# SinclaM/ray-tracer-challenge

Measured on AMD Instinct MI355X. Metric: Mrays/sec (primary+secondary), scenes/cover.json 1920x1080 depth 5, higher is better.
Workload: dtype f64

## Files before the change

### ray-tracer-challenge_amd/csrc/rtc_kernels.hip

```cpp
#include "rtc_device.h"

#include <type_traits>

#if defined(RTC_PROFILE) && defined(RTC_PROFILE_LITE)
#define RTC_STAMP(sec)                                                     \
  do {                                                                     \
    if ((sec) == 7) prof_t = __builtin_amdgcn_s_memtime();                 \
    (void)prof_sec;                                                        \
  } while (0)
#define RTC_COUNT(slot) do { } while (0)
#define RTC_HIST_BEGIN() do { } while (0)
#define RTC_HIST_END(kind) do { } while (0)
#elif defined(RTC_PROFILE)
#define RTC_STAMP(sec)                                                     \
  do {                                                                     \
    const unsigned long long now_ = __builtin_amdgcn_s_memtime();          \
    prof_acc[prof_sec] += now_ - prof_t;                                   \
    prof_t = now_;                                                         \
    prof_sec = (sec);                                                      \
  } while (0)
#define RTC_COUNT(slot)                                                                 \
  do {                                                                                  \
    prof2[slot] += 1ull;                                                                \
    prof2[(slot) + 1] += static_cast<unsigned long long>(__builtin_popcountll(__ballot(true))); \
// ... 26 lines not shown
    if (__builtin_amdgcn_mbcnt_hi(static_cast<uint32_t>(__ballot(true) >> 32), __builtin_amdgcn_mbcnt_lo(static_cast<uint32_t>(__ballot(true)), 0u)) == 0u) \
      rtc_prof_counts[threadIdx.x >> 6][slot] += n_;                                                                   \
  } while (0)
#define RTC_WALK_ADD(slot, n) RTC_PROF_ADD_(slot, n)
#define RTC_AUX_ADD(slot, n) RTC_PROF_ADD_(8 + (slot), n)
#define RTC_KIND_ADD(slot, n) RTC_PROF_ADD_(16 + (slot), n)
#define RTC_CUBE_ADD(slot, n) RTC_PROF_ADD_(40 + (slot), n)
#else
#define RTC_WALK_ADD(slot, n) do { } while (0)
#define RTC_AUX_ADD(slot, n) do { } while (0)
#define RTC_KIND_ADD(slot, n) do { } while (0)
#define RTC_CUBE_ADD(slot, n) do { } while (0)
#endif

#ifdef RTC_PROFILE
__shared__ uint32_t rtc_oob_avail[6];
__device__ __forceinline__ bool rtc_in_bounds(uint32_t kind, bool ok) {
  if (!ok) atomicAdd(&rtc_prof_stats->oob[kind], 1ull);
  return ok;
}
#define RTC_IN_BOUNDS(kind, ok) rtc_in_bounds(kind, ok)
#define RTC_CHECK_INDEX(kind, i, n) (rtc_in_bounds(kind, (i) < (n)) ? (i) : 0u)
#define RTC_AVAIL(k) rtc_oob_avail[k]
#else
#define RTC_IN_BOUNDS(kind, ok) true
#define RTC_CHECK_INDEX(kind, i, n) (i)
#endif

#ifndef RTC_EXPERIMENT
#define RTC_EXPERIMENT 0
#endif

#ifndef RTC_ROOT_NODE_IN_REC
#define RTC_ROOT_NODE_IN_REC 1
#endif
#ifndef RTC_ALL_SOLID_FORM
#define RTC_ALL_SOLID_FORM 1
#endif
#ifndef RTC_CULL_HALF_STEP
#define RTC_CULL_HALF_STEP 1
#endif
#ifndef RTC_PLANE_EARLY_OUT
#define RTC_PLANE_EARLY_OUT 1
#endif
#ifndef RTC_ROOM_EARLY_OUT
#define RTC_ROOM_EARLY_OUT 1
#endif
#ifndef RTC_CUBE_BEHIND_EARLY_OUT
#define RTC_CUBE_BEHIND_EARLY_OUT 1
#endif
#ifndef RTC_SPECULAR_SKIP
#define RTC_SPECULAR_SKIP 1
#endif
#ifndef RTC_CONTAINERS_SOLIDS
#define RTC_CONTAINERS_SOLIDS 1
#endif
#ifndef RTC_SETPRIO
#define RTC_SETPRIO 1
#endif
#ifndef RTC_PRIO_DEAL
#define RTC_PRIO_DEAL 3
#endif
#ifndef RTC_PRIO_WORK
#define RTC_PRIO_WORK 1
#endif
#ifndef RTC_PRIO_CULL
#define RTC_PRIO_CULL 0
#endif
#ifndef RTC_PRIO_NODE
#define RTC_PRIO_NODE 0
#endif
#ifndef RTC_PRIO_CULL_SPHERES
#define RTC_PRIO_CULL_SPHERES 3
#endif
#if RTC_SETPRIO
#define RTC_PRIO_PHASE(x) __builtin_amdgcn_s_setprio(x)
#else
#define RTC_PRIO_PHASE(x) ((void)0)
#endif
#ifndef RTC_LB2
#define RTC_LB2 2
#endif

namespace {

constexpr double kInf = __builtin_huge_val();

struct Ray {
  double ox, oy, oz, dx, dy, dz;
};

__device__ __forceinline__ double zmax(double a, double b) { return __builtin_fmax(a, b); }
__device__ __forceinline__ double zmin(double a, double b) { return __builtin_fmin(a, b); }

__device__ __forceinline__ double row_pt(const double* __restrict__ m, double x, double y, double z) {
  return ((m[0] * x + m[1] * y) + m[2] * z) + m[3];
}
__device__ __forceinline__ double row_vec(const double* __restrict__ m, double x, double y, double z) {
  return (m[0] * x + m[1] * y) + m[2] * z;
}

__device__ __forceinline__ Ray xform_ray(const double* __restrict__ m, const Ray& r) {
  Ray o;
  o.ox = row_pt(m + 0, r.ox, r.oy, r.oz);
  o.oy = row_pt(m + 4, r.ox, r.oy, r.oz);
  o.oz = row_pt(m + 8, r.ox, r.oy, r.oz);
// ... 1012 lines not shown
                                                   const char* __restrict__ az, const RayB& rb) {
  const Float2 nx = *reinterpret_cast<const Float2*>(ax), fx = *reinterpret_cast<const Float2*>(ax + 8);
  const Float2 ny = *reinterpret_cast<const Float2*>(ay), fy = *reinterpret_cast<const Float2*>(ay + 8);
  const Float2 nz = *reinterpret_cast<const Float2*>(az), fz = *reinterpret_cast<const Float2*>(az + 8);
  const Float2 tnx = __builtin_elementwise_fma(nx, Float2(rb.ix), Float2(rb.cnx)), tny = __builtin_elementwise_fma(ny, Float2(rb.iy), Float2(rb.cny)),
               tnz = __builtin_elementwise_fma(nz, Float2(rb.iz), Float2(rb.cnz));
  const Float2 tfx = __builtin_elementwise_fma(fx, Float2(rb.ix), Float2(rb.cfx)), tfy = __builtin_elementwise_fma(fy, Float2(rb.iy), Float2(rb.cfy)),
               tfz = __builtin_elementwise_fma(fz, Float2(rb.iz), Float2(rb.cfz));
  uint32_t kept = 0u;
#pragma unroll
  for (int e = 0; e < 2; ++e) {
    const float tn = fmaxf(fmaxf(tnx[e], tny[e]), tnz[e]), tf = fminf(fminf(tfx[e], tfy[e]), tfz[e]);
    bool culled = fmaxf(tn, rb.t_lo) > fminf(tf, rb.t_hi);
    if constexpr (GROUPS) {
      const float line_only = (*reinterpret_cast<const Float2*>(pair + 72))[e];
      culled = line_only != 0.0f ? tn > tf : culled;
    }
    kept |= culled ? 0u : (1u << e);
  }
  return kept;
}

template <class V, bool GROUPS>
__device__ __forceinline__ uint32_t roots_kept_box4(const char* __restrict__ pair, const char* __restrict__ ax, const char* __restrict__ ay,
                                                    const char* __restrict__ az, const RayB& rb) {
  constexpr uint32_t NEXT = sizeof(RootBoxPair);
  const Float2 nx[2] = {*reinterpret_cast<const Float2*>(ax), *reinterpret_cast<const Float2*>(ax + NEXT)};
  const Float2 fx[2] = {*reinterpret_cast<const Float2*>(ax + 8), *reinterpret_cast<const Float2*>(ax + NEXT + 8)};
  const Float2 ny[2] = {*reinterpret_cast<const Float2*>(ay), *reinterpret_cast<const Float2*>(ay + NEXT)};
  const Float2 fy[2] = {*reinterpret_cast<const Float2*>(ay + 8), *reinterpret_cast<const Float2*>(ay + NEXT + 8)};
  const Float2 nz[2] = {*reinterpret_cast<const Float2*>(az), *reinterpret_cast<const Float2*>(az + NEXT)};
  const Float2 fz[2] = {*reinterpret_cast<const Float2*>(az + 8), *reinterpret_cast<const Float2*>(az + NEXT + 8)};
  uint32_t kept = 0u;
#pragma unroll
  for (int r = 0; r < 2; ++r) {
    const Float2 tnx = __builtin_elementwise_fma(nx[r], Float2(rb.ix), Float2(rb.cnx)), tny = __builtin_elementwise_fma(ny[r], Float2(rb.iy), Float2(rb.cny)),
                 tnz = __builtin_elementwise_fma(nz[r], Float2(rb.iz), Float2(rb.cnz));
    const Float2 tfx = __builtin_elementwise_fma(fx[r], Float2(rb.ix), Float2(rb.cfx)), tfy = __builtin_elementwise_fma(fy[r], Float2(rb.iy), Float2(rb.cfy)),
                 tfz = __builtin_elementwise_fma(fz[r], Float2(rb.iz), Float2(rb.cfz));
#pragma unroll
    for (int e = 0; e < 2; ++e) {
      const float tn = fmaxf(fmaxf(tnx[e], tny[e]), tnz[e]), tf = fminf(fminf(tfx[e], tfy[e]), tfz[e]);
      bool culled = fmaxf(tn, rb.t_lo) > fminf(tf, rb.t_hi);
      if constexpr (GROUPS) {
        const float line_only = (*reinterpret_cast<const Float2*>(pair + r * NEXT + 72))[e];
        culled = line_only != 0.0f ? tn > tf : culled;
      }
      kept |= culled ? 0u : (1u << (2 * r + e));
    }
  }
  return kept;
}

template <class V>
__device__ __forceinline__ void motion_root(V&, uint32_t) {}

template <bool CSG, int WORLD, class V, int TRAV = RTC_LDS_TRAV, bool BOX = true, bool MOTION = false>
__device__ __forceinline__ void trace(const DevScene& S, const RootRec* __restrict__ recs,
                                      const CullTables& cull, const Ray& ray, V& vis, unsigned& overflow,
                                      uint32_t* lds_stack, const uint32_t member = 0u, const uint32_t stride = 1u,
                                      const double* __restrict__ disp = nullptr, const double tm = 0.0) {
  constexpr bool SIMPLE = WORLD == 2, FLAT = WORLD >= 1;
  static_assert(!MOTION || WORLD == 0, "the motion kernels walk the general world");
  constexpr bool kSolids = SIMPLE && RTC_CONTAINERS_SOLIDS && V::kBehindOnly;
  const auto rf = [&]() {
    if constexpr (BOX) {
      RayB b = ray_box(ray, S, vis);
      if constexpr (kSolids) b.t_lo = -1.0002e-4f;
      return b;
    } else {
      return ray_f32(ray, S.cull_cmax);
    }
  }();
  const uint32_t n_bounded = S.n_roots - S.n_root_planes;
  for (uint32_t base = 0; base < S.n_roots; base += 64u) {
    const uint32_t n = min(64u, S.n_roots - base);
    const uint32_t nc = n_bounded > base ? min(n, n_bounded - base) : 0u;
    unsigned long long mine = 0ull;
    RTC_PRIO_PHASE(BOX ? RTC_PRIO_CULL : RTC_PRIO_CULL_SPHERES);
    if (BOX && FLAT && stride == 1u) {
      if constexpr (BOX) {
        const char* block = reinterpret_cast<const char*>(cull.box + (base >> 1));
        const char* ax = block + rf.onx;
        const char* ay = block + rf.ony;
        const char* az = block + rf.onz;
#if RTC_CULL_HALF_STEP
        const uint32_t whole = (nc & 3u) > 2u ? nc : (nc & ~3u);
#else
        const uint32_t whole = nc;
#endif
#ifdef RTC_PROFILE
        const bool reads_ok = RTC_IN_BOUNDS(RTC_OOB_ROOTS, (base >> 1) + 2u * ((whole + 3u) >> 2) + (whole < nc ? 1u : 0u) <= RTC_AVAIL(2));
#else
        constexpr bool reads_ok = true;
#endif
#pragma unroll 1
        for (uint32_t first = 0; reads_ok && first < whole; first += 4u) {
          const uint32_t k = roots_kept_box4<V, !FLAT>(block, ax, ay, az, rf);
          mine |= static_cast<unsigned long long>(k) << first;
          block += 2u * sizeof(RootBoxPair);
          ax += 2u * sizeof(RootBoxPair);
          ay += 2u * sizeof(RootBoxPair);
          az += 2u * sizeof(RootBoxPair);
        }
#if RTC_CULL_HALF_STEP
        if (reads_ok && whole < nc) mine |= static_cast<unsigned long long>(roots_kept_box<V, !FLAT>(block, ax, ay, az, rf)) << whole;
#endif
      }
    } else {
      for (uint32_t i = 4u * member; i < nc; i += 4u * stride) {
#ifdef RTC_PROFILE
        if (!RTC_IN_BOUNDS(RTC_OOB_ROOTS, ((base + i) >> 1) + ((BOX && !(i + 2u < nc)) ? 1u : 2u) <= RTC_AVAIL(BOX ? 2 : 1))) continue;
#endif
        unsigned long long k;
        if constexpr (BOX) {
          const char* const p0 = reinterpret_cast<const char*>(cull.box + ((base + i) >> 1));
          const char* const p1 = p0 + sizeof(RootBoxPair);
          k = roots_kept_box<V, !FLAT>(p0, p0 + rf.onx, p0 + rf.ony, p0 + rf.onz, rf);
          if (i + 2u < nc) k |= roots_kept_box<V, !FLAT>(p1, p1 + rf.onx, p1 + rf.ony, p1 + rf.onz, rf) << 2;
        } else {
          const RootCullPair p0 = cull.sphere[(base + i) >> 1], p1 = cull.sphere[((base + i) >> 1) + 1u];
          k = roots_kept<V, !FLAT, kSolids>(p0, rf) | (roots_kept<V, !FLAT, kSolids>(p1, rf) << 2);
        }
        mine |= k << i;
      }
    }
    if (nc < 64u) mine &= (1ull << nc) - 1ull;
    if (nc < n) {
      unsigned long long planes = (n < 64u ? (1ull << n) - 1ull : ~0ull) & ~((1ull << nc) - 1ull);
      if (stride != 1u) {
        unsigned long long own = 0xFull << (4u * member);
        if (stride == 4u) own |= own << 16;
        own |= own << 32;
        planes &= own;
      }
      mine |= planes;
    }
    RTC_PRIO_PHASE(RTC_PRIO_WORK);
    auto range = [&](uint32_t lo, uint32_t hi) -> unsigned long long {
      const uint32_t a = max(lo, base) - base, b = min(max(hi, base), base + 64u) - base;
      const unsigned long long below_b = b >= 64u ? ~0ull : (1ull << b) - 1ull;
      const unsigned long long below_a = a >= 64u ? ~0ull : (1ull << a) - 1ull;
      return below_b & ~below_a;
    };
#if defined(RTC_PROFILE) && !defined(RTC_PROFILE_LITE)
    uint32_t cube_tests = 0u, cube_neg = 0u, cube_pred = 0u;
#endif
    constexpr bool kCubeBehind = SIMPLE && BOX && V::kAnyHit && V::kFrontOnly && RTC_CUBE_BEHIND_EARLY_OUT;
    auto leaf_of_kind = [&](auto kind_tag, const uint32_t root) {
      constexpr uint32_t KIND = decltype(kind_tag)::value;
      const RootRec& R = recs[RTC_CHECK_INDEX(RTC_OOB_ROOTS, root, RTC_AVAIL(0))];
      const uint32_t kf = R.kind_flags;
      const Ray lr = xform_ray(R.inv, ray);
      const CylParams cy{0.0, 0.0, false};
      const uint32_t leaf = R.index, shadow = (kf >> 8) & 1u, material = R.material;
      vis.set_root(root);
      if constexpr (KIND == 2u && V::kAnyHit && RTC_ROOM_EARLY_OUT) {
        if ((kf & RTC_ROOT_ROOM) && segment_stays_inside_cube(lr, vis.t_limit())) return;
      }
#if defined(RTC_PROFILE) && !defined(RTC_PROFILE_LITE)
      if constexpr (KIND == 2u) {
        double c_tmin, c_tmax;
        cube_slab(lr, c_tmin, c_tmax);
        const bool neg = c_tmax < 0.0, pred = cube_entirely_behind(lr);
        constexpr uint32_t K = V::kAnyHit ? 6u : (V::kBehindOnly ? 12u : 0u);
        RTC_CUBE_ADD(K + 0u, __builtin_popcountll(__ballot(true)));
        RTC_CUBE_ADD(K + 1u, __builtin_popcountll(__ballot(neg)));
        RTC_CUBE_ADD(K + 2u, __builtin_popcountll(__ballot(pred)));
        RTC_CUBE_ADD(K + 3u, 1);
        cube_neg += neg ? 1u : 0u;
        cube_pred += pred ? 1u : 0u;
        cube_tests += 1u;
      }
#endif
      if constexpr (KIND == 2u && kCubeBehind) {
        if (cube_entirely_behind(lr)) return;
      }
      if constexpr (KIND == 1u && V::kFrontOnly && RTC_PLANE_EARLY_OUT) {
        if (__builtin_fabs(lr.dy) > 1e-5) {
          const double ao = __builtin_fabs(lr.oy), ad = __builtin_fabs(lr.dy);
          const bool negative = ((lr.oy > 0.0) == (lr.dy > 0.0)) & (ao >= 1e-290) & (ad <= 1e10);
          const bool beyond = ao > (vis.t_limit() * ad) * (1.0 + 1e-12);
          if (!(negative | beyond)) vis.entry(leaf, shadow, material, -lr.oy / lr.dy, 0.0, 0.0);
        }
      } else if constexpr (KIND == 1u && kSolids) {
        if (__builtin_fabs(lr.dy) > 1e-5 && (lr.oy > 0.0) == (lr.dy > 0.0)) vis.entry(leaf, shadow, material, -lr.oy / lr.dy, 0.0, 0.0);
      } else {
        leaf_entries<SIMPLE>(KIND, cy, nullptr, lr, [&](double t, double u, double v) { vis.entry(leaf, shadow, material, t, u, v); });
      }
    };
    auto leaves_of_kind = [&](auto kind_tag, unsigned long long m) {
      while (m != 0ull && !vis.done()) {
        const uint32_t bit = static_cast<uint32_t>(__builtin_ctzll(m));
        m &= m - 1ull;
        if constexpr (V::kBehindOnly) RTC_AUX_ADD(4, 1);
        leaf_of_kind(kind_tag, base + bit);
      }
    };
    if constexpr (FLAT) {
      const uint32_t k1 = S.n_root_spheres, k2 = k1 + S.n_root_cubes;
      if (stride == 1u) {
        const uint32_t p1 = base + n;
        for (uint32_t root = base + nc; root < p1; ++root) {
          if (__all(vis.done())) break;
          if constexpr (V::kBehindOnly) RTC_AUX_ADD(4, 1);
          if (!vis.done()) leaf_of_kind(std::integral_constant<uint32_t, 1u>{}, root);
        }

      } else {
        leaves_of_kind(std::integral_constant<uint32_t, 1u>{}, mine & range(n_bounded, S.n_roots));
      }
      leaves_of_kind(std::integral_constant<uint32_t, 0u>{}, mine & range(0u, k1));
      leaves_of_kind(std::integral_constant<uint32_t, 2u>{}, mine & range(k1, k2));
#if defined(RTC_PROFILE) && !defined(RTC_PROFILE_LITE)
      {
        constexpr uint32_t K = V::kAnyHit ? 6u : (V::kBehindOnly ? 12u : 0u);
        uint32_t left_neg = 0u, left_pred = 0u;
        while (__ballot(cube_tests - cube_neg > left_neg) != 0ull) ++left_neg;
        while (__ballot(cube_tests - cube_pred > left_pred) != 0ull) ++left_pred;
        RTC_CUBE_ADD(K + 4u, left_neg);
        RTC_CUBE_ADD(K + 5u, left_pred);
      }
#endif
      if constexpr (SIMPLE) continue;
      mine &= range(k2, n_bounded);
    }
    while (mine != 0ull && !vis.done()) {
      const uint32_t bit = static_cast<uint32_t>(__builtin_ctzll(mine));
      mine &= mine - 1ull;
      const RootRec& R = recs[RTC_CHECK_INDEX(RTC_OOB_ROOTS, base + bit, RTC_AVAIL(0))];
      const uint32_t kf = R.kind_flags;
      Ray shifted;
      if constexpr (MOTION) {
        const double* __restrict__ D = disp + 3ull * (base + bit);
        shifted = ray;
        shifted.ox = ray.ox - tm * D[0];
        shifted.oy = ray.oy - tm * D[1];
        shifted.oz = ray.oz - tm * D[2];
        motion_root(vis, base + bit);
      }
      const Ray& root_ray = MOTION ? shifted : ray;
      if (FLAT || !(kf & RTC_ROOT_IS_GROUP)) {
        if (!FLAT && V::kShadowOnly && ((kf >> 8) & 1u) == 0u) continue;
        const Ray lr = xform_ray(R.inv, root_ray);
        if constexpr (V::kAnyHit && RTC_ROOM_EARLY_OUT) {
          if ((kf & RTC_ROOT_ROOM) && segment_stays_inside_cube(lr, vis.t_limit())) continue;
        }
// ... 984 lines not shown
#ifdef RTC_GLOSS_TU
  static_assert(GLOSS, "the gloss translation unit compiles the gloss kernels only: its Pending carries the path code");
#else
  static_assert(!GLOSS, "rough materials are compiled in the gloss translation unit (rtc_gloss.hip) only");
  (void)gloss;
#endif
  static_assert(!OCCL || GLOSS, "the occlusion kernels are the gloss walk");
#ifdef RTC_OCCL_TU
  static_assert(OCCL, "the occlusion translation unit compiles the occlusion kernels only");
#else
  static_assert(!OCCL, "ambient occlusion is compiled in the occlusion translation unit (rtc_occlusion.hip) only");
  (void)occl;
#endif
  static_assert(!SFILT || OCCL, "the shadow-filter kernels are the occlusion walk");
#ifdef RTC_SFILT_TU
  static_assert(SFILT, "the shadow-filter translation unit compiles the shadow-filter kernels only");
#else
  static_assert(!SFILT, "shadow filters are compiled in the shadow-filter translation unit (rtc_shadowfilter.hip) only");
  (void)sfilt;
#endif
  static_assert(!MEDIA || SFILT, "the media kernels are the shadow-filter walk");
#ifdef RTC_MEDIA_TU
  static_assert(MEDIA, "the media translation unit compiles the media kernels only: its Pending carries a medium and three weights");
#else
  static_assert(!MEDIA, "participating media are compiled in the media translation unit (rtc_media.hip) only");
  (void)media;
#endif
  RTC_PRIO_PHASE(RTC_PRIO_WORK);
#ifndef RTC_PROFILE
  if (blockIdx.x == 0u) {
    uint32_t* z = reinterpret_cast<uint32_t*>(next_stats);
    for (uint32_t i = threadIdx.x; i < sizeof(DevStats) / sizeof(uint32_t); i += blockDim.x) z[i] = 0u;
  }
#else
  (void)next_stats;
  if (threadIdx.x == 0u) rtc_prof_stats = stats;
#ifndef RTC_PROFILE_LITE
  for (uint32_t i = threadIdx.x; i < 4u * 58u; i += blockDim.x) rtc_prof_counts[i / 58u][i % 58u] = 0ull;
#endif
  __syncthreads();
#endif
  constexpr int N_ROOTS = WAVES == 3 ? RTC_LDS3_ROOTS : RTC_LDS_ROOTS, N_MATS = WAVES == 3 ? RTC_LDS3_MATERIALS : RTC_LDS_MATERIALS,
                N_PATS = WAVES == 3 ? RTC_LDS3_PATTERNS : RTC_LDS_PATTERNS;
  __shared__ RootRec lds_recs[LDS ? N_ROOTS : 1];
  __shared__ RootCullPair lds_cull[(LDS && !BOX) ? N_ROOTS / 2 : 1];
  __shared__ RootBoxPair lds_box[(LDS && BOX) ? N_ROOTS / 2 : 1];
  __shared__ DevMaterial lds_mat[LDS ? N_MATS : 1];
  __shared__ DevPattern lds_pat[LDS ? N_PATS : 1];
  constexpr int N_LIGHTS = WAVES == 3 ? RTC_LDS3_LIGHTS : RTC_LDS_LIGHTS;
  __shared__ double lds_light[LDS ? 6 * N_LIGHTS : 1];
  __shared__ uint4 lds_mail[4][64];
  constexpr bool SIMPLE = WORLD == 2, FLAT = WORLD >= 1;
  constexpr bool kSpecularSkip = SIMPLE && RTC_SPECULAR_SKIP;
  constexpr int LDS_LEVELS = (FLAT || !LDS) ? 2 : 1;
  __shared__ Quad2 lds_pend[4][LDS_LEVELS][4][64];
  __shared__ double lds_acc[4][64][3];
  constexpr int TRAV = (WAVES == 3 && RTC_BVH8) ? 2 : ((MEDIA && LDS && !FLAT) ? RTC_LDS_TRAV - 2 : RTC_LDS_TRAV);
  __shared__ uint32_t lds_trav[FLAT ? 1 : 4][FLAT ? 1 : TRAV][RTC_BVH8 ? 128 : 64];
  const RootRec* __restrict__ recs = S.root_recs;
  CullTables cull{S.root_cull, S.root_box};
  const DevMaterial* __restrict__ mats = S.mat;
  const DevPattern* __restrict__ pats = S.pat;
  const double* __restrict__ lights = S.light;
  const double* __restrict__ area_rows = AREA ? area.row : nullptr;
#ifdef RTC_PROFILE
  uint32_t area_avail = AREA ? RTC_AREA_ROW * S.n_lights : 0u;
#endif
  if (LDS) {
    auto stage = [&](void* dst_, const void* src_, uint32_t n_words) {
      const double* __restrict__ src = reinterpret_cast<const double*>(src_);
      double* dst = reinterpret_cast<double*>(dst_);
      for (uint32_t i = threadIdx.x; i < n_words; i += blockDim.x) dst[i] = src[i];
    };
#ifndef RTC_PROFILE
    stage(lds_recs, S.root_recs, S.n_roots * (sizeof(RootRec) / 8u));
    if constexpr (BOX) stage(lds_box, S.root_box, ((S.n_roots + 7u) & ~7u) / 2u * (sizeof(RootBoxPair) / 8u));
    else stage(lds_cull, S.root_cull, ((S.n_roots + 3u) & ~3u) / 2u * (sizeof(RootCullPair) / 8u));
    stage(lds_mat, S.mat, S.n_materials * (sizeof(DevMaterial) / 8u));
    stage(lds_pat, S.pat, S.n_patterns * (sizeof(DevPattern) / 8u));
    stage(lds_light, S.light, S.n_lights * 6u);
#else
    auto words = [&](uint32_t n, size_t src_words, size_t dst_words) -> uint32_t {
      const uint32_t m = static_cast<uint32_t>(min(static_cast<size_t>(n), min(src_words, dst_words)));
      if (threadIdx.x == 0u) (void)RTC_IN_BOUNDS(RTC_OOB_STAGING, m == n);
      return m;
    };
    constexpr uint32_t W_REC = sizeof(RootRec) / 8u, W_CULL = sizeof(RootCullPair) / 8u, W_BOX = sizeof(RootBoxPair) / 8u,
                       W_MAT = sizeof(DevMaterial) / 8u, W_PAT = sizeof(DevPattern) / 8u;
    const uint32_t w_recs = words(S.n_roots * W_REC, static_cast<size_t>(S.n_root_recs) * W_REC, sizeof lds_recs / 8u);
    stage(lds_recs, S.root_recs, w_recs);
    uint32_t w_box = 0u, w_cull = 0u;
    if constexpr (BOX) {
      w_box = words(((S.n_roots + 7u) & ~7u) / 2u * W_BOX, static_cast<size_t>(S.n_root_box) * W_BOX, sizeof lds_box / 8u);
      stage(lds_box, S.root_box, w_box);
    } else {
      w_cull = words(((S.n_roots + 3u) & ~3u) / 2u * W_CULL, static_cast<size_t>(S.n_root_cull) * W_CULL, sizeof lds_cull / 8u);
      stage(lds_cull, S.root_cull, w_cull);
    }
    const uint32_t w_mat = words(S.n_materials * W_MAT, static_cast<size_t>(S.n_materials) * W_MAT, sizeof lds_mat / 8u);
    stage(lds_mat, S.mat, w_mat);
    const uint32_t w_pat = words(S.n_patterns * W_PAT, static_cast<size_t>(S.n_patterns) * W_PAT, sizeof lds_pat / 8u);
    stage(lds_pat, S.pat, w_pat);
    const uint32_t w_light = words(S.n_lights * 6u, static_cast<size_t>(S.n_lights) * 6u, sizeof lds_light / 8u);
    stage(lds_light, S.light, w_light);
    if (threadIdx.x == 0u) {
      rtc_oob_avail[0] = w_recs / W_REC;
// ... 389 lines not shown
      const unsigned long long live = __ballot(have_cur);
      const uint32_t n_live = static_cast<uint32_t>(__builtin_popcountll(live));
      coop = n_live <= 8u;
      if (coop) {
        uint32_t src = 0u;
        unsigned long long m = live;
        for (uint32_t k = 0; k < n_live; ++k) {
          const uint32_t b = static_cast<uint32_t>(__builtin_ctzll(m));
          m &= m - 1ull;
          if ((lane >> 3) == k) src = b;
        }
        yield_from = 8u * bits_below(live);
        Pending w;
        w.ray = {__shfl(cur.ray.ox, src), __shfl(cur.ray.oy, src), __shfl(cur.ray.oz, src),
                 __shfl(cur.ray.dx, src), __shfl(cur.ray.dy, src), __shfl(cur.ray.dz, src)};
        w.weight = __shfl(cur.weight, src);
        w.remaining = __shfl(cur.remaining, src);
        cur = w;
        work = (lane >> 3) < n_live;
        member = lane & 7u;
        stride = 8u;
      }
    }
    if constexpr (!COOP) {
      if (!have_cur) continue;
    }
    have_cur = false;
    unsigned& it_share = COOP ? yield.share : share_rays;
    unsigned& it_secondary = COOP ? yield.secondary : n_secondary;
    unsigned& it_shadow_calls = COOP ? yield.shadow_calls : n_shadow_calls;
    unsigned& it_shadow_traced = COOP ? yield.shadow_traced : n_shadow_traced;
    unsigned& it_overflow = COOP ? yield.overflow : overflow;
    if (work) do {
    it_share += 2u;
    cur.remaining = min(cur.remaining, max_depth);
    const Ray ray = cur.ray;
    double tm = 0.0;
    if constexpr (MOTION) {
      uint32_t px, py;
      map_pixel(map, out_index, px, py);
      const unsigned long long p = static_cast<unsigned long long>(py) * cam.hsize + px;
      tm = rtc_camera_jitter(smp.key, p, smp.sample_base + (*samp_word & RTC_SAMPLE_MASK), RTC_MOTION_AXIS);
    }

    RTC_STAMP(1);
#ifdef RTC_PROFILE
    prof_iters += 1ull;
#endif
    using HitVisitor = typename std::conditional<MOTION, MotionClosestVisitor, ClosestVisitor>::type;
    HitVisitor hv;
    RTC_COUNT(0);
    {
      RTC_HIST_BEGIN();
      trace<CSG, WORLD, HitVisitor, TRAV, BOX, MOTION>(S, recs, cull, ray, hv, it_overflow, trav_stack, member, stride, mo.disp, tm);
      RTC_HIST_END(0);
    }
    RTC_STAMP(2);
#ifdef RTC_MEDIA_TU
    if constexpr (MEDIA) {
      const bool atmosphere = cur.medium == RTC_NO_MEDIUM;
      double s_r = media.fog_density, s_g = media.fog_density, s_b = media.fog_density;
      if (!atmosphere) {
        const double* __restrict__ A = media.absorption + 3ull * cur.medium;
        s_r = A[0];
        s_g = A[1];
        s_b = A[2];
      }
      double t_r = 1.0, t_g = 1.0, t_b = 1.0;
      if (__any(s_r != 0.0 || s_g != 0.0 || s_b != 0.0)) {
        if (hv.leaf != RTC_NO_LEAF) {
          const double dist = hv.t * __builtin_sqrt((ray.dx * ray.dx + ray.dy * ray.dy) + ray.dz * ray.dz);
          t_r = s_r == 0.0 ? 1.0 : exp(-(s_r * dist));
          t_g = s_g == 0.0 ? 1.0 : exp(-(s_g * dist));
          t_b = s_b == 0.0 ? 1.0 : exp(-(s_b * dist));
        } else {
          t_r = s_r == 0.0 ? 1.0 : 0.0;
          t_g = s_g == 0.0 ? 1.0 : 0.0;
          t_b = s_b == 0.0 ? 1.0 : 0.0;
        }
      }
      if (atmosphere && media.fog_density > 0.0) {
        acc[0] = acc[0] + cur.weight * ((1.0 - t_r) * media.fog_color[0]);
        acc[1] = acc[1] + cur.weight_g * ((1.0 - t_g) * media.fog_color[1]);
        acc[2] = acc[2] + cur.weight_b * ((1.0 - t_b) * media.fog_color[2]);
      }
      cur.weight = cur.weight * t_r;
      cur.weight_g = cur.weight_g * t_g;
      cur.weight_b = cur.weight_b * t_b;
    }
    uint32_t kid_medium = RTC_NO_MEDIUM;
#endif
    if (hv.leaf == RTC_NO_LEAF) continue;

    uint32_t kind, geom, mat_index;
    double M_copy[FLAT ? 12 : 1];
    const double* M = M_copy;
    DevCyl hcy{0.0, 0.0, 0u, 0u};
    if (FLAT || hv.root != RTC_NO_LEAF) {
      const RootRec& R = recs[RTC_CHECK_INDEX(RTC_OOB_ROOTS, hv.root, RTC_AVAIL(0))];
      if constexpr (FLAT) {
#pragma unroll
        for (int i = 0; i < 12; ++i) M_copy[i] = R.inv[i];
      } else {
        M = R.inv;
      }
      kind = R.kind_flags & 0xFFu;
      geom = R.geom;
      mat_index = R.material;
      hcy.ymin = R.ymin;
      hcy.ymax = R.ymax;
    } else {
      const uint4 meta = S.leaf_meta[hv.leaf];
      M = S.xf + 12ull * meta.y;
      kind = meta.x & 0xFFu;
      geom = meta.w;
      mat_index = meta.z;
      if (RTC_HAS_CYL_ROW(kind)) hcy = S.cyl[geom];
    }
#ifdef RTC_PROFILE
    mat_index = RTC_CHECK_INDEX(RTC_OOB_MATERIALS, mat_index, RTC_AVAIL(3));
#endif
    RTC_STAMP(10);
    const double t = hv.t;
    double n1 = 1.0, n2 = 1.0;
    if (cur.remaining != 0u && !(mats[mat_index].transparency == 0.0)) {
      RTC_STAMP(5);
      it_share += 2u;
      using BehindVisitor = BehindVisitorT<WORLD == 2>;
      BehindVisitor bv;
      bv.hit_leaf = hv.leaf;
      bv.hit_t = t;
      RTC_COUNT(4);
      RTC_AUX_ADD(7, 1);
      {
        RTC_HIST_BEGIN();
        trace<CSG, WORLD, BehindVisitor, TRAV, BOX, MOTION>(S, recs, cull, ray, bv, it_overflow, trav_stack, member, stride, mo.disp, tm);
        RTC_HIST_END(2);
      }
        RTC_STAMP(6);
      bv.template flush<true>();
      const double hit_ior = mats[mat_index].ior;
      if (bv.best_leaf != RTC_NO_LEAF) n1 = mats[RTC_CHECK_INDEX(RTC_OOB_MATERIALS, bv.best_mat, RTC_AVAIL(3))].ior;
      if (!bv.hit_open) {
        n2 = hit_ior;
      } else if (bv.best_excl_leaf != RTC_NO_LEAF) {
        n2 = mats[RTC_CHECK_INDEX(RTC_OOB_MATERIALS, bv.best_excl_mat, RTC_AVAIL(3))].ior;
      } else if (bv.hit_dups >= 2u) {
        n2 = hit_ior;
      }
#ifdef RTC_MEDIA_TU
      kid_medium = !bv.hit_open ? mat_index : (bv.best_excl_leaf != RTC_NO_LEAF ? bv.best_excl_mat : (bv.hit_dups >= 2u ? mat_index : RTC_NO_MEDIUM));
#endif
    }
    const double ptx = ray.ox + ray.dx * t, pty = ray.oy + ray.dy * t, ptz = ray.oz + ray.dz * t;
    const double ex = -ray.dx, ey = -ray.dy, ez = -ray.dz;
    double spx = ptx, spy = pty, spz = ptz, mdx = 0.0, mdy = 0.0, mdz = 0.0;
    if constexpr (MOTION) {
      const double* __restrict__ D = mo.disp + 3ull * hv.hit_root;
      mdx = D[0];
      mdy = D[1];
      mdz = D[2];
      spx = ptx - tm * mdx;
      spy = pty - tm * mdy;
      spz = ptz - tm * mdz;
    }
    const double lpx = row_pt(M + 0, spx, spy, spz);
    const double lpy = row_pt(M + 4, spx, spy, spz);
    const double lpz = row_pt(M + 8, spx, spy, spz);
    double lnx, lny, lnz;
    switch (SIMPLE ? min(kind, 2u) : kind) {
      case 0:
        lnx = lpx;
        lny = lpy;
        lnz = lpz;
        break;
      case 1:
        lnx = 0.0;
        lny = 1.0;
        lnz = 0.0;
        break;
      case 2: {
        const double ax = __builtin_fabs(lpx), ay = __builtin_fabs(lpy), az = __builtin_fabs(lpz);
        const double maxc = zmax(ax, zmax(ay, az));
        lnx = lny = lnz = 0.0;
        if (maxc == ax) {
          lnx = lpx;
        } else if (maxc == ay) {
          lny = lpy;
        } else {
// ... 86 lines not shown
        const double qy = row_pt(R + 4, lpx, lpy, lpz);
        const double qz = row_pt(R + 8, lpx, lpy, lpz);
        double d0, d1, d2;
        if (bump_kind == 1.0) {
          const uint32_t octaves = static_cast<uint32_t>(R[15]);
          const double persistence = R[13];
          d0 = octave_noise(qx, qy, qz, octaves, persistence);
          d1 = octave_noise(qx, qy, qz + 1.0, octaves, persistence);
          d2 = octave_noise(qx, qy, qz + 2.0, octaves, persistence);
        } else {
          d1 = 0.0;
          bump_ripples(qx, qz, d0, d2);
        }
        const double amp = R[12];
        const double bx = lnx / lmag + d0 * amp, by = lny / lmag + d1 * amp, bz = lnz / lmag + d2 * amp;
        hx = (M[0] * bx + M[4] * by) + M[8] * bz;
        hy = (M[1] * bx + M[5] * by) + M[9] * bz;
        hz = (M[2] * bx + M[6] * by) + M[10] * bz;
        const double mag = __builtin_sqrt((hx * hx + hy * hy) + hz * hz);
        if (mag != 0.0) {
          hx = hx / mag;
          hy = hy / mag;
          hz = hz / mag;
        }
        if (inside) {
          hx = -hx;
          hy = -hy;
          hz = -hz;
        }
      }
    }
    RTC_STAMP(11);
    const double eps = 1e-5;
    const double ovx = ptx + nx * eps, ovy = pty + ny * eps, ovz = ptz + nz * eps;
#ifdef RTC_OCCL_TU
    double occl_ka = mats[mat_index].ambient;
    if constexpr (OCCL) {
      const double occl_radius = occl.row[mat_index];
      if (occl_radius > 0.0 && occl_ka != 0.0) {
        uint32_t opx, opy;
        map_pixel(map, out_index, opx, opy);
        const unsigned long long occl_h = rtc_gloss_sample_key(
            occl.key, static_cast<unsigned long long>(opy) * cam.hsize + opx,
            static_cast<unsigned long long>(smp.sample_base) + (*samp_word & RTC_SAMPLE_MASK));
        uint32_t clear = 0u;
        for (uint32_t k = 0u; k < occl.samples; ++k) {
          const GlossDir od = occl_direction(occl_h, (k << RTC_OCCLUSION_SAMPLE_SHIFT) | cur.code, nx, ny, nz);
          it_shadow_calls++;
          it_shadow_traced++;
          it_share++;
          ShadowVisitor sv;
          sv.distance = occl_radius;
          Ray sray{ovx, ovy, ovz, od.x, od.y, od.z};
          trace<CSG, WORLD, ShadowVisitor, TRAV, BOX, MOTION>(S, recs, cull, sray, sv, it_overflow, trav_stack, member, stride, mo.disp, tm);
          clear += sv.shadowed ? 0u : 1u;
        }
        if (clear != occl.samples) occl_ka = occl_ka * (static_cast<double>(clear) / static_cast<double>(occl.samples));
      }
    }
#endif
    double sr = 0.0, sg = 0.0, sb = 0.0;
    {
      const DevMaterial& mat = mats[mat_index];
      constexpr bool SOLID_PATH = RTC_ALL_SOLID_FORM != 0 && !(WORLD == 2 && !BOX);
      Rgb color;
      if (SOLID_PATH && S.all_solid != 0u) {
        const DevPattern& P = pats[RTC_CHECK_INDEX(RTC_OOB_PATTERNS, mat.pattern, RTC_AVAIL(4))];
        color = {P.rgb[0], P.rgb[1], P.rgb[2]};
      } else {
        double qx = ovx, qy = ovy, qz = ovz;
        if constexpr (MOTION) {
          qx = ovx - tm * mdx;
          qy = ovy - tm * mdy;
          qz = ovz - tm * mdz;
        }
        const double opx = row_pt(M + 0, qx, qy, qz);
        const double opy = row_pt(M + 4, qx, qy, qz);
        const double opz = row_pt(M + 8, qx, qy, qz);
#ifdef RTC_MESHUV_TU
        const MeshUvHit mh{muv.row, ((kind == 4u || kind == 5u) && muv.row != nullptr) ? geom : RTC_NO_LEAF, hv.u, hv.v};
#endif
        color = pattern_at<CSG>(S, pats, RTC_CHECK_INDEX(RTC_OOB_PATTERNS, mat.pattern, RTC_AVAIL(4)), opx, opy, opz RTC_MESHUV_ARG);
      }
      RTC_STAMP(12);
      const bool shadow_matters = !(mat.diffuse == 0.0 && mat.specular == 0.0);
      const bool deal_lights = COOP && coop && S.n_lights <= 2u;
      const uint32_t li_first = deal_lights ? (member >> 2) : 0u, li_step = deal_lights ? 2u : 1u;
      const uint32_t s_member = deal_lights ? (member & 3u) : member, s_stride = deal_lights ? 4u : stride;
      const unsigned calls_before = it_shadow_calls, traced_before = it_shadow_traced, share_before = it_share;
      for (uint32_t li = li_first; li < S.n_lights; li += li_step) {
#ifdef RTC_PROFILE
        if (!RTC_IN_BOUNDS(RTC_OOB_LIGHTS, 6u * li + 6u <= RTC_AVAIL(5))) continue;
        if (AREA && !RTC_IN_BOUNDS(RTC_OOB_LIGHTS, RTC_AREA_ROW * li + RTC_AREA_ROW <= area_avail)) continue;
#endif
        if constexpr (AREA) {
          const double* __restrict__ A = area_rows + static_cast<size_t>(RTC_AREA_ROW) * li;
          const unsigned long long bits = static_cast<unsigned long long>(__double_as_longlong(A[12]));
          if ((bits >> RTC_AREA_KIND_BIT) & 1ull) {
            const uint32_t us = static_cast<uint32_t>(bits) & ((1u << RTC_AREA_STEP_BITS) - 1u);
            const uint32_t vs = static_cast<uint32_t>(bits >> RTC_AREA_STEP_BITS) & ((1u << RTC_AREA_STEP_BITS) - 1u);
            const bool jitter = (bits >> RTC_AREA_JITTER_BIT) & 1ull;
            const uint32_t n_samples = us * vs;
            it_shadow_calls += n_samples;
            unsigned long long pixel = 0ull;
            if (jitter) {
              uint32_t px, py;
              if (map.mode == 0u) {
// ... 30 lines not shown
            double lr_ = er * ka, lg_ = eg * ka, lb_ = eb * ka;
            double dr = 0.0, dg = 0.0, db = 0.0;
            if (shadow_matters) {
              for (uint32_t v = 0u; v < vs; ++v)
                for (uint32_t u = 0u; u < us; ++u) {
                  double vx, vy, vz;
                  to_sample(u, v, vx, vy, vz);
                  const double distance = __builtin_sqrt((vx * vx + vy * vy) + vz * vz);
                  double lvx = vx, lvy = vy, lvz = vz;
                  if (distance != 0.0) {
                    lvx = vx / distance;
                    lvy = vy / distance;
                    lvz = vz / distance;
                  }
                  const double light_dot_normal = (lvx * hx + lvy * hy) + lvz * hz;
                  if (light_dot_normal >= 0.0) {
                    const double kd = mat.diffuse * light_dot_normal;
                    dr = dr + er * kd;
                    dg = dg + eg * kd;
                    db = db + eb * kd;
                    const double two_dot = 2.0 * light_dot_normal;
                    const double rx = lvx - hx * two_dot, ry = lvy - hy * two_dot, rz = lvz - hz * two_dot;
                    const double reflect_dot_eye = ((-rx) * ex + (-ry) * ey) + (-rz) * ez;
                    if (reflect_dot_eye > 0.0) {
                      const uint32_t n = mat.shininess_int;
                      const double ks = mat.specular * (n != 0u && reflect_dot_eye < kInf ? pow_small_int(reflect_dot_eye, n)
                                                                                          : zig_pow(reflect_dot_eye, mat.shininess));
                      dr = dr + A[9] * ks;
                      dg = dg + A[10] * ks;
                      db = db + A[11] * ks;
                    }
                  }
                }
            }
            if (!(dr == 0.0 && dg == 0.0 && db == 0.0)) {
              RTC_LIT_DECL;
              for (uint32_t v = 0u; v < vs; ++v)
                for (uint32_t u = 0u; u < us; ++u) {
                  double vx, vy, vz;
                  to_sample(u, v, vx, vy, vz);
                  const double distance = __builtin_sqrt((vx * vx + vy * vy) + vz * vz);
                  double lvx = vx, lvy = vy, lvz = vz;
                  if (distance != 0.0) {
                    lvx = vx / distance;
                    lvy = vy / distance;
                    lvz = vz / distance;
                  }
                  it_shadow_traced++;
                  it_share++;
                  RTC_LIGHT_VISITOR sv;
                  sv.distance = distance;
                  RTC_LIGHT_VISITOR_SET(sv);
                  Ray sray{ovx, ovy, ovz, lvx, lvy, lvz};
                  trace<CSG, WORLD, RTC_LIGHT_VISITOR, TRAV, BOX, MOTION>(S, recs, cull, sray, sv, it_overflow, trav_stack, member, stride, mo.disp, tm);
                  RTC_LIT_ADD(sv);
                }
              const double samples = static_cast<double>(n_samples);
              RTC_LIT_INTENSITY(samples);
              lr_ = lr_ + (dr / samples) * RTC_INTENSITY(r);
              lg_ = lg_ + (dg / samples) * RTC_INTENSITY(g);
              lb_ = lb_ + (db / samples) * RTC_INTENSITY(b);
            }
            sr = sr + lr_;
            sg = sg + lg_;
            sb = sb + lb_;
            continue;
          }
        }
        const double* __restrict__ L = lights + 6ull * li;
        if constexpr (!SPOT) it_shadow_calls++;
        const double vx = L[0] - ovx, vy = L[1] - ovy, vz = L[2] - ovz;
        const double distance = __builtin_sqrt((vx * vx + vy * vy) + vz * vz);
        double lvx = vx, lvy = vy, lvz = vz;
        if (distance != 0.0) {
          lvx = vx / distance;
          lvy = vy / distance;
          lvz = vz / distance;
        }
        const double light_dot_normal = (lvx * hx + lvy * hy) + lvz * hz;
        bool shadowed = false;
        RTC_SF_DECL;
        double spot_f = 1.0;
        if constexpr (SPOT) {
          typedef const __attribute__((address_space(4))) double ConstRow;
          ConstRow* C = (ConstRow*)spots.row + static_cast<size_t>(RTC_SPOT_ROW) * __builtin_amdgcn_readfirstlane(li);
          if (C[5] != 0.0) spot_f = rtc_spot_factor(-((lvx * C[0] + lvy * C[1]) + lvz * C[2]), C[3], C[4]);
          shadowed = spot_f == 0.0;
          if (!shadowed) it_shadow_calls++;
        }
        if (!shadowed && shadow_matters && light_dot_normal >= 0.0 && !(RTC_EXPERIMENT & 1)) {
          it_shadow_traced++;
          it_share++;
          RTC_LIGHT_VISITOR sv;
          sv.distance = distance;
          RTC_LIGHT_VISITOR_SET(sv);
          Ray sray{ovx, ovy, ovz, lvx, lvy, lvz};
          RTC_STAMP(3);
          RTC_COUNT(2);
          {
            RTC_HIST_BEGIN();
            trace<CSG, WORLD, RTC_LIGHT_VISITOR, TRAV, BOX, MOTION>(S, recs, cull, sray, sv, it_overflow, trav_stack, s_member, s_stride, mo.disp, tm);
            RTC_HIST_END(1);
          }
                RTC_STAMP(4);
          shadowed = RTC_LIGHT_BLOCKED(sv);
          RTC_SF_TAKE(sv);
        }
        const double er = color.r * L[3], eg = color.g * L[4], eb = color.b * L[5];
        const double ka = RTC_KA(mat);
        double lr_ = er * ka, lg_ = eg * ka, lb_ = eb * ka;
        if (!shadowed) {
          double dr = 0.0, dg = 0.0, db = 0.0, pr = 0.0, pg = 0.0, pb = 0.0;
          if (light_dot_normal >= 0.0) {
            const double kd = mat.diffuse * light_dot_normal;
            dr = er * kd;
            dg = eg * kd;
            db = eb * kd;
            if constexpr (SPOT) {
              dr = dr * spot_f;
              dg = dg * spot_f;
              db = db * spot_f;
            }
            const double two_dot = 2.0 * light_dot_normal;
            const double rx = lvx - hx * two_dot, ry = lvy - hy * two_dot, rz = lvz - hz * two_dot;
            const double reflect_dot_eye = ((-rx) * ex + (-ry) * ey) + (-rz) * ez;
            if (reflect_dot_eye > 0.0) {
              const uint32_t n = mat.shininess_int;
              bool ks_is_specular = false;
              if (mat.specular == 0.0) ks_is_specular = n != 0u && reflect_dot_eye <= 1.0;
#ifdef RTC_PROFILE
              {
                const unsigned long long lanes_ = static_cast<unsigned long long>(__builtin_popcountll(__ballot(true)));
                const unsigned long long idle_ = __ballot(!ks_is_specular) == 0ull ? 1ull : 0ull;
                RTC_AUX_ADD(li != 0u ? 1 : 0, 1ull + (idle_ << 32));
                RTC_AUX_ADD(li != 0u ? 3 : 2, lanes_ + ((idle_ * lanes_) << 32));
              }
#endif
              double ks = mat.specular;
              if (!(kSpecularSkip && ks_is_specular))
                ks = mat.specular * (n != 0u && reflect_dot_eye < kInf ? pow_small_int(reflect_dot_eye, n)
                                                                       : zig_pow(reflect_dot_eye, mat.shininess));
              pr = L[3] * ks;
              pg = L[4] * ks;
              pb = L[5] * ks;
              if constexpr (SPOT) {
                pr = pr * spot_f;
                pg = pg * spot_f;
                pb = pb * spot_f;
              }
            }
          }
          lr_ = (lr_ + RTC_SF(dr, r)) + RTC_SF(pr, r);
          lg_ = (lg_ + RTC_SF(dg, g)) + RTC_SF(pg, g);
          lb_ = (lb_ + RTC_SF(db, b)) + RTC_SF(pb, b);
// ... 1117 lines not shown
```

Measured before the change: 16780.

## Use 32-bit root masks with carry-chain bit assembly in three-wave simple kernels

Adds a 32-root specialization of trace for the simple world, three-wave box kernels. Root masks become 32-bit instead of 64-bit, and the cull loop walks the box records backwards. Each loop step builds the kept bits by shifting compare results into the mask with inline v_addc carry-chain assembly instead of shift-and-or. The aim is fewer VGPRs and ALU instructions in the hot cull loop. The cost is hand-written assembly with a hard-coded s_nop hazard wait, and the path only works when the scene has at most 32 roots.

```diff
diff --git a/ray-tracer-challenge_amd/csrc/rtc_kernels.hip b/ray-tracer-challenge_amd/csrc/rtc_kernels.hip
--- a/ray-tracer-challenge_amd/csrc/rtc_kernels.hip
+++ b/ray-tracer-challenge_amd/csrc/rtc_kernels.hip
@@ -102,6 +102,9 @@
 #ifndef RTC_SPECULAR_SKIP
 #define RTC_SPECULAR_SKIP 1
 #endif
+#ifndef RTC_ROOTS32
+#define RTC_ROOTS32 1
+#endif
 #ifndef RTC_CONTAINERS_SOLIDS
 #define RTC_CONTAINERS_SOLIDS 1
 #endif
@@ -1220,15 +1223,62 @@
   return kept;
 }
 
+template <class V, int RECORDS>
+__device__ __forceinline__ uint32_t roots_shifted_in_box(uint32_t m, const char* __restrict__ ax, const char* __restrict__ ay,
+                                                         const char* __restrict__ az, const RayB& rb) {
+  constexpr uint32_t NEXT = sizeof(RootBoxPair);
+  static_assert(RECORDS == 1 || RECORDS == 2, "the half step and the step of four roots");
+  Float2 nx[RECORDS], fx[RECORDS], ny[RECORDS], fy[RECORDS], nz[RECORDS], fz[RECORDS];
+  unsigned long long kept[2 * RECORDS];
+#pragma unroll
+  for (int r = 0; r < RECORDS; ++r) {
+    nx[r] = *reinterpret_cast<const Float2*>(ax + r * NEXT);
+    fx[r] = *reinterpret_cast<const Float2*>(ax + r * NEXT + 8);
+    ny[r] = *reinterpret_cast<const Float2*>(ay + r * NEXT);
+    fy[r] = *reinterpret_cast<const Float2*>(ay + r * NEXT + 8);
+    nz[r] = *reinterpret_cast<const Float2*>(az + r * NEXT);
+    fz[r] = *reinterpret_cast<const Float2*>(az + r * NEXT + 8);
+  }
+#pragma unroll
+  for (int r = RECORDS - 1; r >= 0; --r) {
+    const Float2 tnx = __builtin_elementwise_fma(nx[r], Float2(rb.ix), Float2(rb.cnx)), tny = __builtin_elementwise_fma(ny[r], Float2(rb.iy), Float2(rb.cny)),
+                 tnz = __builtin_elementwise_fma(nz[r], Float2(rb.iz), Float2(rb.cnz));
+    const Float2 tfx = __builtin_elementwise_fma(fx[r], Float2(rb.ix), Float2(rb.cfx)), tfy = __builtin_elementwise_fma(fy[r], Float2(rb.iy), Float2(rb.cfy)),
+                 tfz = __builtin_elementwise_fma(fz[r], Float2(rb.iz), Float2(rb.cfz));
+#pragma unroll
+    for (int e = 1; e >= 0; --e) {
+      const float tn = fmaxf(fmaxf(tnx[e], tny[e]), tnz[e]), tf = fminf(fminf(tfx[e], tfy[e]), tfz[e]);
+      kept[2 * r + e] = __builtin_amdgcn_fcmpf(fmaxf(tn, rb.t_lo), fminf(tf, rb.t_hi), 13);
+    }
+  }
+  if constexpr (RECORDS == 2) {
+    asm("s_nop 1\n\t"
+        "v_addc_co_u32_e64 %0, vcc, %0, %0, %1\n\t"
+        "v_addc_co_u32_e64 %0, vcc, %0, %0, %2\n\t"
+        "v_addc_co_u32_e64 %0, vcc, %0, %0, %3\n\t"
+        "v_addc_co_u32_e64 %0, vcc, %0, %0, %4"
+        : "+v"(m) : "s"(kept[3]), "s"(kept[2]), "s"(kept[1]), "s"(kept[0]) : "vcc");
+  } else {
+    asm("s_nop 1\n\t"
+        "v_addc_co_u32_e64 %0, vcc, %0, %0, %1\n\t"
+        "v_addc_co_u32_e64 %0, vcc, %0, %0, %2"
+        : "+v"(m) : "s"(kept[1]), "s"(kept[0]) : "vcc");
+  }
+  return m;
+}
+
 template <class V>
 __device__ __forceinline__ void motion_root(V&, uint32_t) {}
 
-template <bool CSG, int WORLD, class V, int TRAV = RTC_LDS_TRAV, bool BOX = true, bool MOTION = false>
+template <bool CSG, int WORLD, class V, int TRAV = RTC_LDS_TRAV, bool BOX = true, bool MOTION = false, int MAX_ROOTS = 64>
 __device__ __forceinline__ void trace(const DevScene& S, const RootRec* __restrict__ recs,
                                       const CullTables& cull, const Ray& ray, V& vis, unsigned& overflow,
                                       uint32_t* lds_stack, const uint32_t member = 0u, const uint32_t stride = 1u,
                                       const double* __restrict__ disp = nullptr, const double tm = 0.0) {
   constexpr bool SIMPLE = WORLD == 2, FLAT = WORLD >= 1;
+  constexpr bool R32 = MAX_ROOTS == 32;
+  static_assert(MAX_ROOTS == 64 || (R32 && SIMPLE && RTC_LDS3_ROOTS == 32), "the 32-root form is the three-wave simple kernels'");
+  using Mask = std::conditional_t<R32, uint32_t, unsigned long long>;
   static_assert(!MOTION || WORLD == 0, "the motion kernels walk the general world");
   constexpr bool kSolids = SIMPLE && RTC_CONTAINERS_SOLIDS && V::kBehindOnly;
   const auto rf = [&]() {
@@ -1241,10 +1291,11 @@
     }
   }();
   const uint32_t n_bounded = S.n_roots - S.n_root_planes;
-  for (uint32_t base = 0; base < S.n_roots; base += 64u) {
-    const uint32_t n = min(64u, S.n_roots - base);
-    const uint32_t nc = n_bounded > base ? min(n, n_bounded - base) : 0u;
-    unsigned long long mine = 0ull;
+  [[maybe_unused]] const auto below32 = [](uint32_t x) -> uint32_t { return x >= 32u ? ~0u : (1u << x) - 1u; };
+  for (uint32_t base = 0; base < (R32 ? 1u : S.n_roots); base += 64u) {
+    const uint32_t n = R32 ? S.n_roots : min(64u, S.n_roots - base);
+    const uint32_t nc = R32 ? n_bounded : (n_bounded > base ? min(n, n_bounded - base) : 0u);
+    Mask mine = 0u;
     RTC_PRIO_PHASE(BOX ? RTC_PRIO_CULL : RTC_PRIO_CULL_SPHERES);
     if (BOX && FLAT && stride == 1u) {
       if constexpr (BOX) {
@@ -1262,25 +1313,42 @@
 #else
         constexpr bool reads_ok = true;
 #endif
+        if constexpr (R32) {
+          const uint32_t steps = (whole + 3u) >> 2;
+          ax += steps * (2u * static_cast<uint32_t>(sizeof(RootBoxPair)));
+          ay += steps * (2u * static_cast<uint32_t>(sizeof(RootBoxPair)));
+          az += steps * (2u * static_cast<uint32_t>(sizeof(RootBoxPair)));
+#if RTC_CULL_HALF_STEP
+          if (reads_ok && whole < nc) mine = roots_shifted_in_box<V, 1>(mine, ax, ay, az, rf);
+#endif
 #pragma unroll 1
-        for (uint32_t first = 0; reads_ok && first < whole; first += 4u) {
-          const uint32_t k = roots_kept_box4<V, !FLAT>(block, ax, ay, az, rf);
-          mine |= static_cast<unsigned long long>(k) << first;
-          block += 2u * sizeof(RootBoxPair);
-          ax += 2u * sizeof(RootBoxPair);
-          ay += 2u * sizeof(RootBoxPair);
-          az += 2u * sizeof(RootBoxPair);
-        }
+          for (uint32_t step = steps; reads_ok && step != 0u; --step) {
+            ax -= 2u * sizeof(RootBoxPair);
+            ay -= 2u * sizeof(RootBoxPair);
+            az -= 2u * sizeof(RootBoxPair);
+            mine = roots_shifted_in_box<V, 2>(mine, ax, ay, az, rf);
+          }
+        } else {
+#pragma unroll 1
+          for (uint32_t first = 0; reads_ok && first < whole; first += 4u) {
+            const uint32_t k = roots_kept_box4<V, !FLAT>(block, ax, ay, az, rf);
+            mine |= static_cast<unsigned long long>(k) << first;
+            block += 2u * sizeof(RootBoxPair);
+            ax += 2u * sizeof(RootBoxPair);
+            ay += 2u * sizeof(RootBoxPair);
+            az += 2u * sizeof(RootBoxPair);
+          }
 #if RTC_CULL_HALF_STEP
-        if (reads_ok && whole < nc) mine |= static_cast<unsigned long long>(roots_kept_box<V, !FLAT>(block, ax, ay, az, rf)) << whole;
-#endif
+          if (reads_ok && whole < nc) mine |= static_cast<unsigned long long>(roots_kept_box<V, !FLAT>(block, ax, ay, az, rf)) << whole;
+#endif
+        }
       }
     } else {
       for (uint32_t i = 4u * member; i < nc; i += 4u * stride) {
 #ifdef RTC_PROFILE
         if (!RTC_IN_BOUNDS(RTC_OOB_ROOTS, ((base + i) >> 1) + ((BOX && !(i + 2u < nc)) ? 1u : 2u) <= RTC_AVAIL(BOX ? 2 : 1))) continue;
 #endif
-        unsigned long long k;
+        Mask k;
         if constexpr (BOX) {
           const char* const p0 = reinterpret_cast<const char*>(cull.box + ((base + i) >> 1));
           const char* const p1 = p0 + sizeof(RootBoxPair);
@@ -1293,23 +1361,33 @@
         mine |= k << i;
       }
     }
-    if (nc < 64u) mine &= (1ull << nc) - 1ull;
+    if constexpr (R32) {
+      mine &= below32(nc);
+    } else {
+      if (nc < 64u) mine &= (1ull << nc) - 1ull;
+    }
     if (nc < n) {
-      unsigned long long planes = (n < 64u ? (1ull << n) - 1ull : ~0ull) & ~((1ull << nc) - 1ull);
+      Mask planes;
+      if constexpr (R32) planes = below32(n) & ~below32(nc);
+      else planes = (n < 64u ? (1ull << n) - 1ull : ~0ull) & ~((1ull << nc) - 1ull);
       if (stride != 1u) {
-        unsigned long long own = 0xFull << (4u * member);
+        Mask own = Mask{0xFu} << (4u * member);
         if (stride == 4u) own |= own << 16;
-        own |= own << 32;
+        if constexpr (!R32) own |= own << 32;
         planes &= own;
       }
       mine |= planes;
     }
     RTC_PRIO_PHASE(RTC_PRIO_WORK);
-    auto range = [&](uint32_t lo, uint32_t hi) -> unsigned long long {
-      const uint32_t a = max(lo, base) - base, b = min(max(hi, base), base + 64u) - base;
-      const unsigned long long below_b = b >= 64u ? ~0ull : (1ull << b) - 1ull;
-      const unsigned long long below_a = a >= 64u ? ~0ull : (1ull << a) - 1ull;
-      return below_b & ~below_a;
+    auto range = [&](uint32_t lo, uint32_t hi) -> Mask {
+      if constexpr (R32) {
+        return below32(hi) & ~below32(lo);
+      } else {
+        const uint32_t a = max(lo, base) - base, b = min(max(hi, base), base + 64u) - base;
+        const unsigned long long below_b = b >= 64u ? ~0ull : (1ull << b) - 1ull;
+        const unsigned long long below_a = a >= 64u ? ~0ull : (1ull << a) - 1ull;
+        return below_b & ~below_a;
+      }
     };
 #if defined(RTC_PROFILE) && !defined(RTC_PROFILE_LITE)
     uint32_t cube_tests = 0u, cube_neg = 0u, cube_pred = 0u;
@@ -1357,10 +1435,10 @@
         leaf_entries<SIMPLE>(KIND, cy, nullptr, lr, [&](double t, double u, double v) { vis.entry(leaf, shadow, material, t, u, v); });
       }
     };
-    auto leaves_of_kind = [&](auto kind_tag, unsigned long long m) {
-      while (m != 0ull && !vis.done()) {
-        const uint32_t bit = static_cast<uint32_t>(__builtin_ctzll(m));
-        m &= m - 1ull;
+    auto leaves_of_kind = [&](auto kind_tag, Mask m) {
+      while (m != 0u && !vis.done()) {
+        const uint32_t bit = static_cast<uint32_t>(R32 ? __builtin_ctz(static_cast<uint32_t>(m)) : __builtin_ctzll(m));
+        m &= m - Mask{1u};
         if constexpr (V::kBehindOnly) RTC_AUX_ADD(4, 1);
         leaf_of_kind(kind_tag, base + bit);
       }
@@ -2451,6 +2529,7 @@
   __shared__ uint4 lds_mail[4][64];
   constexpr bool SIMPLE = WORLD == 2, FLAT = WORLD >= 1;
   constexpr bool kSpecularSkip = SIMPLE && RTC_SPECULAR_SKIP;
+  constexpr int ROOTS = (SIMPLE && WAVES == 3 && BOX && RTC_ROOTS32) ? 32 : 64;
   constexpr int LDS_LEVELS = (FLAT || !LDS) ? 2 : 1;
   __shared__ Quad2 lds_pend[4][LDS_LEVELS][4][64];
   __shared__ double lds_acc[4][64][3];
@@ -2946,7 +3025,7 @@
     RTC_COUNT(0);
     {
       RTC_HIST_BEGIN();
-      trace<CSG, WORLD, HitVisitor, TRAV, BOX, MOTION>(S, recs, cull, ray, hv, it_overflow, trav_stack, member, stride, mo.disp, tm);
+      trace<CSG, WORLD, HitVisitor, TRAV, BOX, MOTION, ROOTS>(S, recs, cull, ray, hv, it_overflow, trav_stack, member, stride, mo.disp, tm);
       RTC_HIST_END(0);
     }
     RTC_STAMP(2);
@@ -3028,7 +3107,7 @@
       RTC_AUX_ADD(7, 1);
       {
         RTC_HIST_BEGIN();
-        trace<CSG, WORLD, BehindVisitor, TRAV, BOX, MOTION>(S, recs, cull, ray, bv, it_overflow, trav_stack, member, stride, mo.disp, tm);
+        trace<CSG, WORLD, BehindVisitor, TRAV, BOX, MOTION, 64>(S, recs, cull, ray, bv, it_overflow, trav_stack, member, stride, mo.disp, tm);
         RTC_HIST_END(2);
       }
         RTC_STAMP(6);
@@ -3221,7 +3300,7 @@
           ShadowVisitor sv;
           sv.distance = occl_radius;
           Ray sray{ovx, ovy, ovz, od.x, od.y, od.z};
-          trace<CSG, WORLD, ShadowVisitor, TRAV, BOX, MOTION>(S, recs, cull, sray, sv, it_overflow, trav_stack, member, stride, mo.disp, tm);
+          trace<CSG, WORLD, ShadowVisitor, TRAV, BOX, MOTION, ROOTS>(S, recs, cull, sray, sv, it_overflow, trav_stack, member, stride, mo.disp, tm);
           clear += sv.shadowed ? 0u : 1u;
         }
         if (clear != occl.samples) occl_ka = occl_ka * (static_cast<double>(clear) / static_cast<double>(occl.samples));
@@ -3358,7 +3437,7 @@
                   sv.distance = distance;
                   RTC_LIGHT_VISITOR_SET(sv);
                   Ray sray{ovx, ovy, ovz, lvx, lvy, lvz};
-                  trace<CSG, WORLD, RTC_LIGHT_VISITOR, TRAV, BOX, MOTION>(S, recs, cull, sray, sv, it_overflow, trav_stack, member, stride, mo.disp, tm);
+                  trace<CSG, WORLD, RTC_LIGHT_VISITOR, TRAV, BOX, MOTION, ROOTS>(S, recs, cull, sray, sv, it_overflow, trav_stack, member, stride, mo.disp, tm);
                   RTC_LIT_ADD(sv);
                 }
               const double samples = static_cast<double>(n_samples);
@@ -3405,7 +3484,7 @@
           RTC_COUNT(2);
           {
             RTC_HIST_BEGIN();
-            trace<CSG, WORLD, RTC_LIGHT_VISITOR, TRAV, BOX, MOTION>(S, recs, cull, sray, sv, it_overflow, trav_stack, s_member, s_stride, mo.disp, tm);
+            trace<CSG, WORLD, RTC_LIGHT_VISITOR, TRAV, BOX, MOTION, ROOTS>(S, recs, cull, sray, sv, it_overflow, trav_stack, s_member, s_stride, mo.disp, tm);
             RTC_HIST_END(1);
           }
                 RTC_STAMP(4);
```

Result: faster. 17090, median of 6 (+1.8%).
